# 0xEigenLabs/eigen-zeth

Measured on AMD Instinct MI355X. Metric: goldilocks_ntt_field_elems_per_s, higher is better.
Workload: dtype u64; 1 GPU; forward NTT, natural order in/out, 2^24 rows x 64 columns per GPU (column-major u64), BASELINE configs[3] shape on one GPU; logn=24, cols_per_gpu=64, cols_total=64

## Files before the change

eigen_zeth_amd/csrc/capi.hip:

```cpp
#include <hip/hip_runtime.h>

#include <cstdio>
#include <cstring>
#include <new>
#include <vector>

#include "ctx.hpp"
#include "poseidon_default_table.inc"

extern "C" {

const char *zp_version(void) { return "zethprover-mi355x 0.1 (gfx950)"; }

int32_t zp_device_count(void) {
    int n = 0;
    return hipGetDeviceCount(&n) == hipSuccess ? n : 0;
}

int32_t zp_create(zp_ctx **out, int32_t device) {
    if (!out) return ZP_ERR_ARG;
    *out = nullptr;
    int ndev = 0;
    if (hipGetDeviceCount(&ndev) != hipSuccess || ndev <= 0) return ZP_ERR_HIP;
    if (device < 0 || device >= ndev) return ZP_ERR_ARG;
// ... 341 lines not shown
        u64 a = next(), b = next();
        if (n_bind > 4) a = bind[4];
        if (n_bind > 5) b = bind[5];
        h_pub[4] = a;
        h_pub[5] = b;
        for (size_t i = 0; i < N; i++) {
            fa[i] = a;
            fb[i] = b;
            const u64 t = gl_add(a, b);
            a = b;
            b = t;
        }
        h_pub[6] = fb[N - 1];
        const int k = logn < 16 ? logn : 16;
        const int rep = logn - k;
        h_pub[7] = ((u64)1 << k) - 1;
        for (size_t i = 0; i < N; i++) {
            rv[i] = next() & (((u64)1 << k) - 1);
            tv[i] = (u64)(i >> rep);
            mv[i] = 0;
        }
        for (size_t i = 0; i < N; i++) {
            mv[(size_t)rv[i] << rep] += 1;
            qv[i] = rv[(5 * i + 3) & (N - 1)];
            cv[i] = gl_mul(rv[i], rv[i]);
            dv[i] = gl_add(gl_mul(fa[i], rv[i]), fb[i]);
        }
        return ZP_OK;
    }
    return ZP_ERR_ARG;
}

int32_t zp_ntt_host(zp_ctx *ctx, uint64_t *h_cols, int32_t logn, int32_t W, int32_t inverse) {
    if (!ctx) return ZP_ERR_ARG;
    ZP_BIND(ctx);
    ZP_ARG(ctx, h_cols != nullptr || W == 0, "null host pointer");
    ZP_ARG(ctx, logn >= 0 && logn <= 32 && W >= 0, "logn/W out of range");
    if (W == 0) return ZP_OK;
    const size_t bytes = ((size_t)W << logn) * sizeof(u64);
    void *d = nullptr;
    ZP_TRY(zp_dev_alloc(ctx, bytes, &d));
    int32_t rc = zp_h2d(ctx, d, h_cols, bytes);
    if (rc == ZP_OK) {
        NttRunOpts o;
        rc = zpi_ntt_run(ctx, (u64 *)d, (u64 *)d, logn, W, inverse != 0, o);
    }
    if (rc == ZP_OK) rc = zp_d2h(ctx, h_cols, d, bytes);
    (void)zp_dev_free(ctx, d);
    return rc;
}

int32_t zp_lde_host(zp_ctx *ctx, const uint64_t *h_in, uint64_t *h_out, int32_t logn, int32_t logb,
                    int32_t W, uint64_t shift) {
    if (!ctx) return ZP_ERR_ARG;
    ZP_BIND(ctx);
    ZP_ARG(ctx, (h_in && h_out) || W == 0, "null host pointer");
    ZP_ARG(ctx, logn >= 0 && logb >= 0 && logn + logb <= 32 && W >= 0, "logn/logb/W out of range");
    if (W == 0) return ZP_OK;
    const size_t bin = ((size_t)W << logn) * sizeof(u64), bout = bin << logb;
    void *di = nullptr, *dout = nullptr;
    ZP_TRY(zp_dev_alloc(ctx, bin, &di));
    int32_t rc = zp_dev_alloc(ctx, bout, &dout);
    if (rc == ZP_OK) rc = zp_h2d(ctx, di, h_in, bin);
    if (rc == ZP_OK) rc = zp_lde(ctx, (const uint64_t *)di, (uint64_t *)dout, nullptr, logn, logb, W, shift);
    if (rc == ZP_OK) rc = zp_d2h(ctx, h_out, dout, bout);
    (void)zp_dev_free(ctx, di);
    (void)zp_dev_free(ctx, dout);
    return rc;
}

int32_t zp_set_tuning(zp_ctx *ctx, const char *key, int32_t value) {
    if (!ctx) return ZP_ERR_ARG;
    ZP_ARG(ctx, key != nullptr, "null key");
    if (!strcmp(key, "ntt_logt")) ctx->tune_logt = value;
    else if (!strcmp(key, "ntt_tpw")) ctx->tune_tpw = value;
    else if (!strcmp(key, "ntt_logt9")) ctx->tune_logt9 = value;
    else if (!strcmp(key, "ntt_logt12")) ctx->tune_logt12 = value;
    else if (!strcmp(key, "msm_chunk_log")) ctx->tune_msm_chunk_log = value;
    else if (!strcmp(key, "msm_c")) ctx->tune_msm_c = value;
    else if (!strcmp(key, "ntt_chunk_log")) ctx->tune_ntt_chunk_log = value;
    else if (!strcmp(key, "ntt_maxl")) ctx->tune_ntt_maxl = value;
    else if (!strcmp(key, "ntt_order")) ctx->tune_ntt_order = value;
    else if (!strcmp(key, "ntt_tw1")) ctx->tune_ntt_tw1 = value;
    else if (!strcmp(key, "ntt_limb")) ctx->tune_ntt_limb = value;
    else if (!strcmp(key, "lde_seam")) ctx->tune_lde_seam = value;
    else if (!strcmp(key, "g16_parallel")) ctx->tune_g16_parallel = value;
    else if (!strcmp(key, "seam_tpw")) ctx->tune_seam_tpw = value;
    else if (!strcmp(key, "lde_seam_plans")) ctx->tune_lde_seam_plans = value;
    else if (!strcmp(key, "merkle_top_wave")) ctx->tune_merkle_top_wave = value;
    else if (!strcmp(key, "ntt_small_wave")) ctx->tune_ntt_small_wave = value;
    else if (!strcmp(key, "synth_rowwise")) ctx->tune_synth_rowwise = value;
    else if (!strcmp(key, "p254_scaled")) ctx->tune_p254_scaled = value;
    else if (!strcmp(key, "p254_block")) ctx->tune_p254_block = value;
    else if (!strcmp(key, "fri_fold_lanes")) ctx->tune_fri_fold_lanes = value;
    else if (!strcmp(key, "copy_grid")) ctx->tune_copy_grid = value;
    else if (!strcmp(key, "copy_nt")) ctx->tune_copy_nt = value;
    else if (!strcmp(key, "copy_block")) ctx->tune_copy_block = value;
    else if (!strcmp(key, "copy_unroll")) ctx->tune_copy_unroll = value;
    else if (!strcmp(key, "merkle_coop_log")) ctx->tune_merkle_coop_log = value;
    else if (!strcmp(key, "p254_bulk_log")) ctx->tune_p254_bulk_log = value;
    else if (!strcmp(key, "verify_lane_min")) ctx->tune_verify_lane_min = value;
    else { ctx->err = "unknown tuning key"; return ZP_ERR_ARG; }
    return ZP_OK;
}

int32_t zp_set_profiling(zp_ctx *ctx, int32_t on) {
    if (!ctx) return ZP_ERR_ARG;
    ctx->profiling = on != 0;
    return ZP_OK;
}

int32_t zp_get_pass_timings(zp_ctx *ctx, float *ms, int32_t *radix_log, int32_t cap, int32_t *count) {
    if (!ctx) return ZP_ERR_ARG;
    ZP_BIND(ctx);
    ZP_ARG(ctx, count != nullptr && cap >= 0 && (cap == 0 || (ms && radix_log)), "bad arguments");
    ZP_HIP(ctx, hipStreamSynchronize(ctx->stream));
    int n = 0;
    for (auto &ev : ctx->pass_events) {
        if (n < cap) {
            float t = 0.f;
            ZP_HIP(ctx, hipEventElapsedTime(&t, ev.a, ev.b));
            ms[n] = t;
            radix_log[n] = ev.radix_log;
            n++;
        }
        (void)hipEventDestroy(ev.a);
        (void)hipEventDestroy(ev.b);
    }
    ctx->pass_events.clear();
    *count = n;
    return ZP_OK;
}

int32_t zp_stage_timings(zp_ctx *ctx, char *buf, size_t buflen) {
    if (!ctx) return ZP_ERR_ARG;
    ZP_BIND(ctx);
    ZP_ARG(ctx, buf && buflen > 2, "null buffer");
    ZP_HIP(ctx, hipStreamSynchronize(ctx->stream));
    std::string s = "[";
    bool first = true;
    for (auto &ev : ctx->stage_events) {
        float t = 0.f;
        if (hipEventElapsedTime(&t, ev.a, ev.b) == hipSuccess) {
            char tmp[128];
            snprintf(tmp, sizeof(tmp), "%s{\"stage\": \"%s\", \"ms\": %.4f}", first ? "" : ", ", ev.name, t);
            s += tmp;
            first = false;
        }
        (void)hipEventDestroy(ev.a);
        (void)hipEventDestroy(ev.b);
    }
    ctx->stage_events.clear();
    s += "]";
    ZP_ARG(ctx, s.size() + 1 <= buflen, "buffer too small");
    memcpy(buf, s.c_str(), s.size() + 1);
    return ZP_OK;
}

int32_t zp_ntt_plan_json(zp_ctx *ctx, int32_t logn, char *buf, size_t buflen) {
    if (!ctx) return ZP_ERR_ARG;
    ZP_ARG(ctx, buf && buflen > 0, "null buffer");
    NttPlan *pl;
    ZP_TRY(zpi_get_plan(ctx, logn, false, &pl));
    std::string s = "{\"logn\": " + std::to_string(logn) + ", \"passes\": [";
    for (int i = 0; i < pl->npass; i++) {
        const NttPassShape sh = zpi_plan_pass_shape(ctx, pl, i);
// ... 37 lines not shown
```

eigen_zeth_amd/csrc/ctx.hpp:

```cpp
#pragma once
#include <hip/hip_runtime.h>

#include <map>
#include <string>
#include <vector>

#include "../../include/zeth_prover.h"
#include "gl.hpp"

#define ZP_ROOT32_DEFAULT 1753635133440165772ULL
#define ZP_SHIFT_DEFAULT 49ULL

struct NttPass {
    int L;
    int logPprev;
};

struct NttPlan {
    int logn = 0;
    bool inverse = false;
    int npass = 0;
    NttPass pass[6];
    int lb = 0;
    u64 *d_twl = nullptr;
    u64 *d_twh = nullptr;
    u64 *d_tws = nullptr;
    u64 *d_tw1 = nullptr;
    bool tw1_unavailable = false;
    u64 w16[8];
    u64 ninv = 1;
    int j0inv = 0;
};

struct CosetTable {
    int logn = 0, lb = 0;
    u64 shift = 0, pre = 0;
    u64 *d_lo = nullptr, *d_hi = nullptr;
};

struct ZpG16Cache;
struct zp_ctx {
    int device = 0;
    hipStream_t stream = nullptr;
    hipStream_t own_stream = nullptr;
    std::string err;
    u64 root32 = ZP_ROOT32_DEFAULT;
    u64 coset_shift = ZP_SHIFT_DEFAULT;
    u64 h_rc[360];
    u64 h_mds[144];
    u64 *d_rc = nullptr;
    u32 *d_mds = nullptr;
    bool poseidon_dirty = true;
    bool mds_is_default = false;
    std::map<int, NttPlan> plans;
    std::vector<CosetTable> cosets;
    u64 *scratch[6] = {nullptr, nullptr, nullptr, nullptr, nullptr, nullptr};
    size_t scratch_elems[6] = {0, 0, 0, 0, 0, 0};
    bool ood_valid = false;
    int ood_logn = -1;
    u64 ood_y[3] = {0, 0, 0}, ood_root32 = 0;
    void *pinned = nullptr;
    size_t pinned_bytes = 0;
    zp_ctx *msm_helpers[4] = {nullptr, nullptr, nullptr, nullptr};
    ZpG16Cache *g16_cache = nullptr;
    int num_cu = 256;
    void *msm_arena = nullptr;
    size_t msm_arena_bytes = 0;
    int tune_logt12 = 2;
    int tune_logt = 4, tune_tpw = 2, tune_logt9 = 4;
    int tune_ntt_tw1 = 26;
    int tune_ntt_limb = 0;
    int tune_lde_seam = 1;
    int tune_seam_tpw = 2;
    int tune_copy_grid = 0, tune_copy_nt = 1, tune_copy_block = 0, tune_copy_unroll = 0;
    int tune_lde_seam_plans = 1;
    int tune_g16_parallel = 1;
    int tune_ntt_order = 0;
    int tune_ntt_maxl = 0;
    int tune_ntt_small_wave = 0;
    int tune_fri_fold_lanes = 0;
    int tune_synth_rowwise = 0;
    int tune_p254_block = 0;
    int tune_p254_scaled = 0;
    int tune_merkle_top_wave = 0;
    int tune_merkle_coop_log = 0;
    int tune_ntt_chunk_log = 0;
    int tune_p254_bulk_log = 0;
    int tune_msm_c = 0;
    int tune_verify_lane_min = 0;
    int tune_msm_chunk_log = 0;
    std::multimap<size_t, void *> prove_pool;
    size_t prove_pool_bytes = 0;
    std::map<std::string, u64 *> prove_fixed;
    size_t prove_fixed_bytes = 0;
    std::map<std::string, void *> air_kernels;
    struct DigestEntry { std::vector<uint64_t> words; uint8_t dg[32]; };
    std::vector<DigestEntry> digest_cache;
    std::vector<u64> last_openings;
    bool profiling = false;
    struct PassEv { hipEvent_t a, b; int radix_log; };
    std::vector<PassEv> pass_events;
    struct StageEv { hipEvent_t a, b; const char *name; };
    std::vector<StageEv> stage_events;
};

struct ZpStage {
    zp_ctx *ctx;
    zp_ctx::StageEv ev;
    bool on;
    ZpStage(zp_ctx *c, const char *name) : ctx(c), on(c && c->profiling) {
        if (c) (void)hipSetDevice(c->device);
        if (on) {
            ev.name = name;
            on = hipEventCreate(&ev.a) == hipSuccess && hipEventCreate(&ev.b) == hipSuccess &&
                 hipEventRecord(ev.a, ctx->stream) == hipSuccess;
        }
    }
    ~ZpStage() {
        if (on && hipEventRecord(ev.b, ctx->stream) == hipSuccess) ctx->stage_events.push_back(ev);
    }
};

#define ZP_BIND(ctx) do { if (ctx) (void)hipSetDevice((ctx)->device); } while (0)

#define ZP_HIP(ctx, call)                                                                    \
    do {                                                                                     \
        hipError_t e_ = (call);                                                              \
        if (e_ != hipSuccess) {                                                              \
            (ctx)->err = std::string(#call) + ": " + hipGetErrorString(e_);                  \
            return e_ == hipErrorOutOfMemory ? ZP_ERR_NOMEM : ZP_ERR_HIP;                    \
        }                                                                                    \
    } while (0)

#define ZP_ARG(ctx, cond, msg)                                                               \
    do {                                                                                     \
        if (!(cond)) {                                                                       \
            (ctx)->err = std::string("bad argument: ") + (msg);                              \
            return ZP_ERR_ARG;                                                               \
        }                                                                                    \
    } while (0)

#define ZP_TRY(expr)                                                                         \
    do {                                                                                     \
        int32_t rc_ = (expr);                                                                \
        if (rc_ != ZP_OK) return rc_;                                                        \
    } while (0)

int32_t zpi_scratch(zp_ctx *ctx, int which, size_t elems, u64 **out);
int32_t zpi_pinned(zp_ctx *ctx, size_t bytes, void **out);
int32_t zpi_d2h_small(zp_ctx *ctx, void *h_dst, const void *d_src, size_t bytes);
int32_t zpi_h2d_small(zp_ctx *ctx, void *d_dst, const void *h_src, size_t bytes);
int32_t zpi_upload(zp_ctx *ctx, const std::vector<u64> &h, u64 **d);
// ... 44 lines not shown
```

eigen_zeth_amd/csrc/ntt.hip:

```cpp
#include <hip/hip_runtime.h>

#include <cstring>
#include <string>

#include "ctx.hpp"
#include "wave_xchg.hpp"
#include "gl_asm.hpp"
#include "gl_limb.hpp"

#define ZP_LDG(p) __builtin_nontemporal_load(p)
#define ZP_STG(p, v) __builtin_nontemporal_store(v, p)

namespace {

typedef __attribute__((ext_vector_type(4))) int zp_i32x4;

struct PassArgs {
    const u64 *in;
    u64 *out;
    u64 in_cs, out_cs;
    u64 in_valid;
    const u64 *twl, *twh;
    const u64 *tws;
    const u64 *tw1;
    const u64 *csl, *csh;
    u64 scale;
    int logn, logPprev, lb, cslb;
    int j0inv;
    int flags;
    int ncols;
};

__device__ __forceinline__ constexpr int brev(int x, int bits) {
    int r = 0;
    for (int i = 0; i < bits; i++) r |= ((x >> i) & 1) << (bits - 1 - i);
    return r;
}
__device__ __forceinline__ constexpr int slot_of(int o, int j, int pos, int A) {
    return ((o >> pos) << (pos + A)) | (j << pos) | (o & ((1 << pos) - 1));
}

template <int A1, int A2, int A3, int LOGT>
struct Geo {
    static constexpr int L = A1 + A2 + A3;
    static constexpr int R = 1 << L;
    static constexpr int T = 1 << LOGT;
    static constexpr int LT = LOGT;
    static constexpr int NT = (R * T) / 16;
    static constexpr int J = 1 + (A2 > 0 ? 1 : 0) + (A3 > 0 ? 1 : 0);
    static constexpr int POS1 = L - A1;
    static constexpr int POS2 = L - A1 - A2;
    static constexpr int AJ = (J == 1) ? A1 : (J == 2 ? A2 : A3);
    __device__ static __forceinline__ int kof(int sigma) {
        int k = (sigma >> POS1) & ((1 << A1) - 1);
        if (A2 > 0) k |= ((sigma >> POS2) & ((1 << A2) - 1)) << A1;
        if (A3 > 0) k |= (sigma & ((1 << A3) - 1)) << (A1 + A2);
        return k;
    }
    __device__ static __forceinline__ int sigma_of_k(int k) {
        int s = (k & ((1 << A1) - 1)) << POS1;
        if (A2 > 0) s |= ((k >> A1) & ((1 << A2) - 1)) << POS2;
        if (A3 > 0) s |= (k >> (A1 + A2)) & ((1 << A3) - 1);
        return s;
    }
    __device__ static __forceinline__ int lpos(int sigma, int t) {
        int s2 = sigma;
        if constexpr (LOGT < 4 && A3 > 0) {
            constexpr int GB = 5 - LOGT;
            s2 ^= ((sigma >> POS2) & ((1 << GB) - 1)) ^ (((sigma >> (POS1 + LOGT)) & ((1 << (A1 - LOGT)) - 1)) << 1);
        }
        return (s2 << LOGT) + (t ^ (kof(sigma) & (T - 1)));
    }
};

__device__ __forceinline__ u64 tw_lookup(const u64 *lo, const u64 *hi, int lb, u64 e) {
    u64 a = lo[e & ((1ULL << lb) - 1)];
    u64 b = hi[e >> lb];
    return gl_mul(a, b);
}

__device__ __forceinline__ u64 mul_c16(int e, u64 d) {
    switch (e) {
        case 0: return d;
        case 1: return gl_shl12<1>(d);
        case 2: return gl_shl12<2>(d);
        case 3: return gl_shl12<3>(d);
        case 4: return gl_shl12<4>(d);
        case 5: return gl_shl12<5>(d);
        case 6: return gl_shl12<6>(d);
        default: return gl_shl12<7>(d);
    }
}
template <int A>
__device__ __forceinline__ void dif_shift(u64 *v) {
    static_assert(A >= 2 && A <= 4, "radix 4, 8 or 16");
#pragma unroll
    for (int s = 0; s < A; s++) {
        const int half = 1 << (A - 1 - s);
#pragma unroll
        for (int t = 0; t < (1 << (A - 1)); t += 2) {
            const int i0 = (t / half) * 2 * half + (t % half), i1 = ((t + 1) / half) * 2 * half + ((t + 1) % half);
            gl_bfly2(v[i0], v[i0 + half], v[i1], v[i1 + half]);
            v[i0 + half] = mul_c16((t % half) * (8 / half), v[i0 + half]);
            v[i1 + half] = mul_c16(((t + 1) % half) * (8 / half), v[i1 + half]);
        }
    }
}

__device__ __forceinline__ void lds_barrier() {
    __builtin_amdgcn_fence(__ATOMIC_RELEASE, "workgroup", "local");
    __builtin_amdgcn_s_barrier();
    __builtin_amdgcn_fence(__ATOMIC_ACQUIRE, "workgroup", "local");
}
// ... 46 lines not shown
        case 1: return gl_l4_mul_c16<1>(d);
        case 2: return gl_l4_mul_c16<2>(d);
        case 3: return gl_l4_mul_c16<3>(d);
        case 4: return gl_l4_mul_c16<4>(d);
        case 5: return gl_l4_mul_c16<5>(d);
        case 6: return gl_l4_mul_c16<6>(d);
        default: return gl_l4_mul_c16<7>(d);
    }
}
template <int A>
__device__ __forceinline__ void dif_levels_l4(gl_l4 *x) {
    static_assert(A >= 2 && A <= 4, "radix 4, 8 or 16");
#pragma unroll
    for (int s = 0; s < A; s++) {
        const int half = 1 << (A - 1 - s);
#pragma unroll
        for (int t = 0; t < (1 << (A - 1)); t++) {
            const int i0 = (t / half) * 2 * half + (t % half);
            const gl_l4 a = x[i0], b = x[i0 + half];
            x[i0] = gl_l4_add(a, b);
            x[i0 + half] = mul_c16_l4((t % half) * (8 / half), gl_l4_sub(a, b));
        }
    }
}
template <int A>
__device__ __forceinline__ void dif_shift_l4(const u64 *v, gl_l4 *x) {
#pragma unroll
    for (int i = 0; i < (1 << A); i++) x[i] = gl_l4_from(v[i]);
    dif_levels_l4<A>(x);
}
__device__ __forceinline__ gl_w4 w4_load(const gl_w4 *p) {
    const zp_i32x4 a = *(const zp_i32x4 *)p->lo, b = *(const zp_i32x4 *)p->hi;
    gl_w4 w;
    w.lo[0] = a.x; w.lo[1] = a.y; w.lo[2] = a.z; w.lo[3] = a.w;
    w.hi[0] = b.x; w.hi[1] = b.y; w.hi[2] = b.z; w.hi[3] = b.w;
    return w;
}
__device__ __forceinline__ void w4_store(gl_w4 *p, const u64 w0, const u64 w1, const u64 w2, const u64 w3) {
    i32 l[4], h[4];
    gl_l4_balance(w0, l[0], h[0]);
    gl_l4_balance(w1, l[1], h[1]);
    gl_l4_balance(w2, l[2], h[2]);
    gl_l4_balance(w3, l[3], h[3]);
    zp_i32x4 a = {l[0], l[1], l[2], l[3]}, b = {h[0], h[1], h[2], h[3]};
    *(zp_i32x4 *)p->lo = a;
    *(zp_i32x4 *)p->hi = b;
}
template <typename G, int A, int POS, int ANEXT, int POSNEXT>
__device__ __forceinline__ void exchange2_l4(const gl_l4 *x, u64 *v, u64 *lds, const gl_w4 *twr4, int j0inv, int tid) {
    constexpr int GR = 16 >> A;
#pragma unroll
    for (int g = 0; g < GR; g++) {
        const int gamma = g * G::NT + tid;
        const int t = gamma & (G::T - 1), o = gamma >> G::LT;
        const int rho = o & ((1 << POS) - 1);
#pragma unroll
        for (int p = 0; p < (1 << A); p++) {
            const int kj = (j0inv * brev(p, A)) & ((1 << A) - 1);
            const u64 y = p == 0 ? gl_l4_canon(x[g * (1 << A)]) : gl_l4_mul(x[g * (1 << A) + p], w4_load(twr4 + kj * rho));
            lds[G::lpos(slot_of(o, kj, POS, A), t)] = y;
        }
    }
    lds_barrier();
    exchange_read<G, ANEXT, POSNEXT>(v, lds, tid);
}

template <typename G>
__device__ __forceinline__ void table_copy_out(u64 *v, const u64 *lds, const u64 *twb, u64 *blk, int tid) {
    constexpr int L = G::L, NT = G::NT;
#pragma unroll
    for (int i = 0; i < 16; i++) v[i] = twb[i * NT + tid];
    lds_barrier();
#pragma unroll
    for (int i = 0; i < 16; i += 2) {
        const int ia = i * NT + tid, ib = (i + 1) * NT + tid;
        u64 xa = lds[G::lpos(G::sigma_of_k(ia & ((1 << L) - 1)), ia >> L)];
        u64 xb = lds[G::lpos(G::sigma_of_k(ib & ((1 << L) - 1)), ib >> L)];
        gl_mul2(xa, v[i], xb, v[i + 1]);
        ZP_STG(&blk[ia], xa);
        ZP_STG(&blk[ib], xb);
    }
}

template <int A1, int A2, int A3, int LOGT, bool TRANSPOSE, bool PADDED, int MODE, bool BIG = false, bool LIMB = false>
__global__ void __launch_bounds__((1 << (A1 + A2 + A3 + LOGT)) / 16, LIMB ? 3 : 4)
ntt_pass2_kernel(PassArgs a, int tiles_per_wg) {
    using G = Geo<A1, A2, A3, LOGT>;
    constexpr int L = G::L, R = G::R, T = G::T, NT = G::NT, AJ = G::AJ;
    constexpr int GRJ = 16 >> AJ;
    constexpr int R2 = 1 << (A2 + A3);
    constexpr bool HAS_TAB = !TRANSPOSE && MODE >= 1;
    constexpr bool TWR_LDS = L <= 10;
    constexpr int TPL = (R + NT - 1) / NT;
    extern __shared__ __attribute__((aligned(16))) u64 lds[];
    constexpr int REC = LIMB ? 4 : 1;
    u64 *tab = lds + R * T;
    u64 *twr1 = tab + (HAS_TAB ? R * REC : 0);
    u64 *twr2 = twr1 + R * REC;
    constexpr bool TW1 = TRANSPOSE && MODE == 3;
    static_assert(!LIMB || (TWR_LDS && (TW1 || !TRANSPOSE)), "limb form: LDS twiddle copies, no per-lane twiddle chain");
    u64 col = blockIdx.y, wg_lin = blockIdx.x;
    if constexpr (TW1) {
        const u64 x = blockIdx.x & 7u, j = blockIdx.x >> 3;
        col = j % (u64)a.ncols;
        wg_lin = (j / (u64)a.ncols) * 8 + x;
    }
    const int logNR = a.logn - L;
    const int logP = a.logPprev;
    const u64 N = 1ULL << a.logn;
    const u64 *src = a.in + col * a.in_cs;
    u64 *dst = a.out + col * a.out_cs;
    u64 v[16], vn[16];
    constexpr int NTW = TW1 ? 1 : TRANSPOSE ? (GRJ + 2) : (MODE == 2 ? TPL + 1 : TPL);
    u64 twl_c[NTW], twh_c[NTW], twl_n[NTW], twh_n[NTW];

    constexpr bool small_n = !BIG;
    auto fetch_tile = [&](u64 *r, u64 *tl, u64 *th, u64 u0, int tid) {
        constexpr int GR = 16 >> A1;
        const u64 valid_rows = a.in_valid >> logNR;
#pragma unroll
        for (int g = 0; g < GR; g++) {
            const int gamma = g * NT + tid;
            const int t = gamma & (T - 1), o = gamma >> LOGT;
            const u32 slot0 = (u32)slot_of(o, 0, G::POS1, A1);
            const u32 lane_bytes = (((u32)slot0 << logNR) + (u32)t) << 3;
            const u64 lane_el = ((u64)slot0 << logNR) + (u64)t;
#pragma unroll
            for (int j = 0; j < (1 << A1); j++) {
                const u64 *rowp = src + (((u64)j << G::POS1) << logNR) + u0;
                const u64 *ptr;
                if constexpr (small_n) ptr = (const u64 *)((const char *)rowp + lane_bytes);
                else ptr = rowp + lane_el;
                u64 val;
                if constexpr (PADDED) val = (u64)(slot0 + ((u32)j << G::POS1)) < valid_rows ? (LOGT < 4 ? *ptr : ZP_LDG(ptr)) : 0ULL;
                else val = LOGT < 4 ? *ptr : ZP_LDG(ptr);
                r[g * (1 << A1) + j] = val;
            }
        }
        const u64 lm = (1ULL << a.lb) - 1;
        if constexpr (TW1) {
            (void)tl; (void)th; (void)lm;
        } else if constexpr (TRANSPOSE) {
            const int t = tid & (T - 1);
            const u64 u = u0 + t;
            const int jr = a.j0inv & ((1 << AJ) - 1);
            u64 e[NTW];
#pragma unroll
            for (int g = 0; g < GRJ; g++) e[g] = u * (u64)G::kof(((g * NT + tid) >> LOGT) << AJ);
            e[GRJ] = ((u << (L - AJ)) * (u64)jr) & (N - 1);
            e[GRJ + 1] = (N - ((u << L) & (N - 1))) & (N - 1);
#pragma unroll
            for (int i = 0; i < NTW; i++) { tl[i] = a.twl[e[i] & lm]; th[i] = a.twh[e[i] >> a.lb]; }
        } else {
            if constexpr (MODE >= 1) {
                const u64 e0 = (u0 >> logP) << logP;
#pragma unroll
                for (int j = 0; j < TPL; j++) {
                    const u64 e = (a.flags & 1) ? e0 * (u64)((tid + j * NT) & (R - 1)) : 0;
                    tl[j] = a.twl[e & lm];
                    th[j] = a.twh[e >> a.lb];
                }
            }
            if constexpr (MODE == 2) {
                const u64 c = (u0 + (tid & (T - 1))) & ((1ULL << logP) - 1);
                tl[TPL] = a.csl[c & ((1ULL << a.cslb) - 1)];
                th[TPL] = a.csh[c >> a.cslb];
            }
        }
    };

    u64 wg = wg_lin;
    if constexpr (LOGT < 4 && !TW1) {
        if ((gridDim.x & 7u) == 0) wg = (u64)(blockIdx.x & 7u) * (gridDim.x >> 3) + (blockIdx.x >> 3);
    }
    const u64 tile0 = wg * tiles_per_wg;
    fetch_tile(v, twl_c, twh_c, tile0 << LOGT, threadIdx.x);
    u64 kfac[TPL];
    {
        const int tid0 = threadIdx.x;
        if constexpr (LIMB) {
            for (int e = tid0; e < R; e += NT) {
                const int rot = (a.j0inv * (R / 8)) & (R - 1);
                w4_store((gl_w4 *)twr1 + e, a.tws[e << (12 - L)], a.tws[((e + rot) & (R - 1)) << (12 - L)],
                         a.tws[((e + 2 * rot) & (R - 1)) << (12 - L)], a.tws[((e + 3 * rot) & (R - 1)) << (12 - L)]);
            }
            if constexpr (G::J >= 3) {
                constexpr int L2 = A2 + A3;
                for (int e = tid0; e < R2; e += NT) {
                    const int rot = (a.j0inv * (R2 / 8)) & (R2 - 1);
                    w4_store((gl_w4 *)twr2 + e, a.tws[e << (12 - L2)], a.tws[((e + rot) & (R2 - 1)) << (12 - L2)],
                             a.tws[((e + 2 * rot) & (R2 - 1)) << (12 - L2)], a.tws[((e + 3 * rot) & (R2 - 1)) << (12 - L2)]);
                }
            }
        } else if constexpr (TWR_LDS) {
            if (tid0 < R) twr1[tid0] = a.tws[tid0 << (12 - L)];
            if constexpr (G::J >= 3) {
                if (tid0 < R2) twr2[tid0] = a.tws[tid0 << (12 - (A2 + A3))];
            }
        }
#pragma unroll
        for (int j = 0; j < TPL; j++) {
            kfac[j] = 1;
            if constexpr (HAS_TAB) {
                if (a.flags & 2) kfac[j] = a.scale;
                if constexpr (MODE == 2) {
                    const u64 ek = (u64)((tid0 + j * NT) & (R - 1)) << logP;
                    kfac[j] = gl_mul(kfac[j], gl_mul(a.csl[ek & ((1ULL << a.cslb) - 1)], a.csh[ek >> a.cslb]));
                }
            }
        }
    }
    lds_barrier();
    __builtin_amdgcn_s_waitcnt(0x0F70);
#pragma clang loop unroll(disable)
    for (int it = 0; it < tiles_per_wg; it++) {
        const u64 u0 = (tile0 + it) << LOGT;
        const bool more = it + 1 < tiles_per_wg;
        int tid = threadIdx.x;
        asm volatile("" : "+v"(tid));
        if (more) fetch_tile(vn, twl_n, twh_n, u0 + T, tid);

        const u64 s = TRANSPOSE ? 0 : (u0 >> logP);
        if constexpr (HAS_TAB) {
#pragma unroll
            for (int j = 0; j < TPL; j++)
                if (tid + j * NT < R) {
                    const u64 w = gl_mul(gl_mul(twl_c[j], twh_c[j]), kfac[j]);
                    if constexpr (LIMB) w4_store((gl_w4 *)tab + tid + j * NT, w, gl_shl12<2>(w), gl_shl12<4>(w), gl_shl12<6>(w));
                    else tab[tid + j * NT] = w;
                }
        }
        gl_l4 x[LIMB ? 16 : 1];
        if constexpr (LIMB) {
#pragma unroll
            for (int g = 0; g < (16 >> A1); g++) dif_shift_l4<A1>(v + g * (1 << A1), x + g * (1 << A1));
            exchange2_l4<G, A1, G::POS1, A2, G::POS2>(x, v, lds, (const gl_w4 *)twr1, a.j0inv, tid);
#pragma unroll
            for (int g = 0; g < (16 >> A2); g++) dif_shift_l4<A2>(v + g * (1 << A2), x + g * (1 << A2));
            if constexpr (G::J >= 3) {
                exchange2_l4<G, A2, G::POS2, A3, 0>(x, v, lds, (const gl_w4 *)twr2, a.j0inv, tid);
#pragma unroll
                for (int g = 0; g < (16 >> A3); g++) dif_shift_l4<A3>(v + g * (1 << A3), x + g * (1 << A3));
            }
        } else {
#pragma unroll
        for (int g = 0; g < (16 >> A1); g++) dif_shift<A1>(v + g * (1 << A1));
        exchange2<G, A1, G::POS1, A2, G::POS2, TWR_LDS ? 0 : 12 - L>(v, lds, TWR_LDS ? twr1 : a.tws, a.j0inv, tid);
#pragma unroll
        for (int g = 0; g < (16 >> A2); g++) dif_shift<A2>(v + g * (1 << A2));
        if constexpr (G::J >= 3) {
            exchange2<G, A2, G::POS2, A3, 0, TWR_LDS ? 0 : 12 - (A2 + A3)>(v, lds, TWR_LDS ? twr2 : a.tws, a.j0inv, tid);
#pragma unroll
            for (int g = 0; g < (16 >> A3); g++) dif_shift<A3>(v + g * (1 << A3));
        }
        }
#pragma unroll
        for (int g = 0; g < GRJ; g++) {
            const int gamma = g * NT + tid;
            const int t = gamma & (T - 1), o = gamma >> LOGT;
            const int klow = G::kof(o << AJ);
            if constexpr (TW1) {
                const int jr = a.j0inv & ((1 << AJ) - 1);
#pragma unroll
                for (int i = 0; i < (1 << AJ); i++) {
                    const int kj = (jr * i) & ((1 << AJ) - 1);
                    if constexpr (LIMB) lds[G::lpos(slot_of(o, kj, 0, AJ), t)] = gl_l4_canon(x[g * (1 << AJ) + brev(i, AJ)]);
                    else lds[G::lpos(slot_of(o, kj, 0, AJ), t)] = v[g * (1 << AJ) + brev(i, AJ)];
                }
            } else if constexpr (TRANSPOSE) {
                const int jr = a.j0inv & ((1 << AJ) - 1);
                u64 w = gl_mul(twl_c[g], twh_c[g]);
                const u64 hj = gl_mul(twl_c[GRJ], twh_c[GRJ]);
                const u64 hjd = gl_mul(hj, gl_mul(twl_c[GRJ + 1], twh_c[GRJ + 1]));
#pragma unroll
                for (int i = 0; i < (1 << AJ); i++) {
                    const int p = brev(i, AJ);
                    const int kj = (jr * i) & ((1 << AJ) - 1);
                    u64 x = v[g * (1 << AJ) + p];
                    if (i + 1 < (1 << AJ)) {
                        const bool wrap = ((jr * (i + 1)) >> AJ) != ((jr * i) >> AJ);
                        u64 wn = w;
                        gl_mul2(x, w, wn, wrap ? hjd : hj);
                        w = wn;
                    } else {
                        x = gl_mul1(x, w);
                    }
                    lds[G::lpos(slot_of(o, kj, 0, AJ), t)] = x;
                }
            } else {
                u64 *const sbase = dst + (s << (logP + L)) + (u0 & ((1ULL << logP) - 1));
                const u32 lane_sb = (((u32)klow << logP) + (u32)t) << 3;
                const u64 lane_se = ((u64)klow << logP) + (u64)t;
                u64 cw = 1;
                if constexpr (MODE == 2) cw = gl_mul(twl_c[TPL], twh_c[TPL]);
#pragma unroll
                for (int p = 0; p < (1 << AJ); p += 2) {
                    const int kja = (a.j0inv * brev(p, AJ)) & ((1 << AJ) - 1), kjb = (a.j0inv * brev(p + 1, AJ)) & ((1 << AJ) - 1);
                    const int ka = klow + (kja << (L - AJ)), kb = klow + (kjb << (L - AJ));
                    u64 xa, xb;
                    if constexpr (LIMB) {
                        if constexpr (MODE >= 1) {
                            xa = gl_l4_mul(x[g * (1 << AJ) + p], w4_load((const gl_w4 *)tab + ka));
                            xb = gl_l4_mul(x[g * (1 << AJ) + p + 1], w4_load((const gl_w4 *)tab + kb));
                        } else {
                            xa = gl_l4_canon(x[g * (1 << AJ) + p]);
                            xb = gl_l4_canon(x[g * (1 << AJ) + p + 1]);
                        }
                    } else {
                        xa = v[g * (1 << AJ) + p];
                        xb = v[g * (1 << AJ) + p + 1];
                        if constexpr (MODE >= 1) gl_mul2(xa, tab[ka], xb, tab[kb]);
                    }
                    if constexpr (MODE == 2) gl_mul2(xa, cw, xb, cw);
                    u64 *const ua = sbase + ((u64)(kja << (L - AJ)) << logP), *const ub = sbase + ((u64)(kjb << (L - AJ)) << logP);
                    u64 *pa, *pb;
                    if constexpr (small_n) { pa = (u64 *)((char *)ua + lane_sb); pb = (u64 *)((char *)ub + lane_sb); }
                    else { pa = ua + lane_se; pb = ub + lane_se; }
                    if constexpr (LOGT < 4) {
                        *pa = xa;
                        *pb = xb;
                    } else {
                        ZP_STG(pa, xa);
                        ZP_STG(pb, xb);
                    }
                }
            }
        }
        if constexpr (TW1) {
            table_copy_out<G>(v, lds, a.tw1 + (u0 << L), dst + (u0 << L), tid);
        } else if constexpr (TRANSPOSE) {
            lds_barrier();
            u64 *blk = dst + (u0 << L);
#pragma unroll
            for (int i = 0; i < 16; i++) {
                const int idx = i * NT + tid;
                const int t2 = idx >> L, k = idx & ((1 << L) - 1);
                ZP_STG(&blk[idx], lds[G::lpos(G::sigma_of_k(k), t2)]);
            }
        }
        if (more) {
            lds_barrier();
#pragma unroll
            for (int i = 0; i < 16; i++) v[i] = vn[i];
#pragma unroll
            for (int i = 0; i < NTW; i++) { twl_c[i] = twl_n[i]; twh_c[i] = twh_n[i]; }
        }
    }
}

struct SeamArgs {
    const u64 *in;
    u64 *out;
    u64 *coef;
    const u64 *tws_i, *tws_f;
    const u64 *tw1;
    const u64 *csl, *csh;
    u64 scale;
    int logn, cslb, j0inv_i, j0inv_f, ncols;
};
__global__ void __launch_bounds__(256, 4) lde_seam_kernel(SeamArgs a, int tiles_per_wg) {
    using G = Geo<4, 4, 0, 4>;
    constexpr int L = 8, R = 256, T = 16, LOGT = 4;
    extern __shared__ __attribute__((aligned(16))) u64 lds[];
    u64 *tab = lds + R * T;
    u64 *twr_i = tab + R;
    u64 *twr_f = twr_i + R;
    const u64 x8 = blockIdx.x & 7u, jj = blockIdx.x >> 3;
    const u64 col = jj % (u64)a.ncols, wg = (jj / (u64)a.ncols) * 8 + x8;
    const int logNR = a.logn - L;
    const u64 N = 1ULL << a.logn;
    const u64 *src = a.in + col * N;
    u64 *dst = a.out + col * (2 * N);
    u64 *cdst = a.coef ? a.coef + col * N : nullptr;
    u64 v[16];
    u64 cw_c[2];
    auto fetch_tile = [&](u64 *r, u64 *cwr, u64 u0, int tid) {
        const int t = tid & (T - 1), o = tid >> LOGT;
        const u32 slot0 = (u32)slot_of(o, 0, G::POS1, 4);
        const u32 lane_bytes = (((u32)slot0 << logNR) + (u32)t) << 3;
#pragma unroll
        for (int j = 0; j < 16; j++) {
            const u64 *rowp = src + (((u64)j << G::POS1) << logNR) + u0;
            r[j] = ZP_LDG((const u64 *)((const char *)rowp + lane_bytes));
        }
        const u64 c = u0 + (u64)t;
        cwr[0] = a.csl[c & ((1ULL << a.cslb) - 1)];
        cwr[1] = a.csh[c >> a.cslb];
    };
    const u64 tile0 = wg * tiles_per_wg;
    {
        const int tid0 = threadIdx.x;
        twr_i[tid0] = a.tws_i[tid0 << (12 - L)];
        twr_f[tid0] = a.tws_f[tid0 << (12 - L)];
        const u64 ek = (u64)tid0 << logNR;
        tab[tid0] = gl_mul(a.scale, gl_mul(a.csl[ek & ((1ULL << a.cslb) - 1)], a.csh[ek >> a.cslb]));
    }
    lds_barrier();
#pragma clang loop unroll(disable)
    for (int it = 0; it < tiles_per_wg; it++) {
        const u64 u0 = (tile0 + it) << LOGT;
        int tid = threadIdx.x;
        asm volatile("" : "+v"(tid));
        fetch_tile(v, cw_c, u0, tid);
        const int t = tid & (T - 1), o = tid >> LOGT;
        dif_shift<4>(v);
        exchange2<G, 4, G::POS1, 4, G::POS2, 0>(v, lds, twr_i, a.j0inv_i, tid);
        dif_shift<4>(v);
        const u64 cw = gl_mul(cw_c[0], cw_c[1]);
        lds_barrier();
#pragma unroll
        for (int p = 0; p < 16; p += 2) {
            const int kja = (a.j0inv_i * brev(p, 4)) & 15, kjb = (a.j0inv_i * brev(p + 1, 4)) & 15;
            const int ka = o + (kja << 4), kb = o + (kjb << 4);
            u64 xa = v[p], xb = v[p + 1];
            gl_mul2(xa, tab[ka], xb, tab[kb]);
            gl_mul2(xa, cw, xb, cw);
            if (cdst) {
                ZP_STG((u64 *)((char *)(cdst + ((u64)ka << logNR) + u0) + (t << 3)), xa);
                ZP_STG((u64 *)((char *)(cdst + ((u64)kb << logNR) + u0) + (t << 3)), xb);
            }
            lds[(((ka & 1) << 7) + (ka >> 1)) * T + t] = xa;
            lds[(((kb & 1) << 7) + (kb >> 1)) * T + t] = xb;
        }
        lds_barrier();
        u64 f1[8];
#pragma unroll
        for (int j = 0; j < 8; j++) {
            v[j] = lds[((j << 4) + o) * T + t];
            f1[j] = lds[(128 + (j << 4) + o) * T + t];
        }
// ... 43 lines not shown
    if (!((lane >> LH) & 1)) return gl_add(x, y);
    const u64 d = gl_sub(y, x);
    return i ? gl_mul(d, tws[(u64)i << (12 - (LH + 1))]) : d;
}

template <bool WAVE>
__global__ void __launch_bounds__(256) ntt_small_kernel(SmallArgs a) {
    extern __shared__ __attribute__((aligned(16))) u64 lds[];
    const int tid = threadIdx.x;
    const int n = 1 << a.logn;
    const u64 *src = a.in + (u64)blockIdx.x * a.in_cs;
    u64 *dst = a.out + (u64)blockIdx.x * a.out_cs;
    for (int i = tid; i < n; i += 256) lds[i] = (u64)i < a.in_valid ? src[i] : 0ULL;
    __syncthreads();
    const int lds_stages = WAVE ? (a.logn > 6 ? a.logn - 6 : 0) : a.logn;
    for (int s = 0; s < lds_stages; s++) {
        const int lh = a.logn - 1 - s;
        const int half = 1 << lh;
        for (int b = tid; b < (n >> 1); b += 256) {
            const int i = b & (half - 1);
            const int i0 = ((b >> lh) << (lh + 1)) + i, i1 = i0 + half;
            u64 x = lds[i0], y = lds[i1];
            lds[i0] = gl_add(x, y);
            u64 d = gl_sub(x, y);
            lds[i1] = i ? gl_mul(d, a.tws[(u64)i << (12 - (lh + 1))]) : d;
        }
        __syncthreads();
    }
    if constexpr (WAVE) {
        const int lane = tid & 63;
        for (int base = (tid >> 6) << 6; base < n; base += 256) {
            u64 x = base + lane < n ? lds[base + lane] : 0ULL;
            const int top = a.logn < 6 ? a.logn : 6;
            if (top >= 6) x = wave_stage<5>(x, lane, a.tws);
            if (top >= 5) x = wave_stage<4>(x, lane, a.tws);
            if (top >= 4) x = wave_stage<3>(x, lane, a.tws);
            if (top >= 3) x = wave_stage<2>(x, lane, a.tws);
            if (top >= 2) x = wave_stage<1>(x, lane, a.tws);
            if (top >= 1) x = wave_stage<0>(x, lane, a.tws);
            const int i = base + lane;
            if (i < n) {
                const int k = brev(i, a.logn);
                if (a.flags & 2) x = gl_mul(x, a.scale);
                if (a.flags & 4) x = gl_mul(x, tw_lookup(a.csl, a.csh, a.cslb, (u64)k));
                dst[k] = x;
            }
        }
        return;
    }
    for (int i = tid; i < n; i += 256) {
        const int k = brev(i, a.logn);
        u64 x = lds[i];
        if (a.flags & 2) x = gl_mul(x, a.scale);
        if (a.flags & 4) x = gl_mul(x, tw_lookup(a.csl, a.csh, a.cslb, (u64)k));
        dst[k] = x;
    }
}

__global__ void __launch_bounds__(256) coset_scale_kernel(const u64 *in, u64 *out, u64 n, const u64 *lo,
                                                         const u64 *hi, int lb) {
    const u64 col = blockIdx.y;
    const u64 i = ((u64)blockIdx.x * 256 + threadIdx.x);
    if (i < n) out[col * n + i] = gl_mul(in[col * n + i], tw_lookup(lo, hi, lb, i));
}

__global__ void __launch_bounds__(256) twiddle_rows_kernel(u64 *rows, int logn_row, u64 total, u64 row0, u64 nmask,
                                                           const u64 *lo, const u64 *hi, int lb) {
    const u64 i = (u64)blockIdx.x * 256 + threadIdx.x;
    if (i >= total) return;
    const u64 r = i >> logn_row, k = i & ((1ULL << logn_row) - 1);
    const u64 e = ((row0 + r) * k) & nmask;
    rows[i] = gl_mul(rows[i], tw_lookup(lo, hi, lb, e));
}

__global__ void __launch_bounds__(256) tw1_fill_kernel(u64 *out, int logn, int L, const u64 *lo, const u64 *hi, int lb) {
    const u64 i = (u64)blockIdx.x * 256 + threadIdx.x;
    if (i >> logn) return;
    const u64 u = i >> L, k = i & ((1ULL << L) - 1);
    out[i] = tw_lookup(lo, hi, lb, (u * k) & ((1ULL << logn) - 1));
}

using PassKernel = void (*)(PassArgs, int);

template <int A1, int A2, int A3, int LOGT, bool BIG>
PassKernel pick_pass_kernel(bool transpose, bool table, bool padded, int mode, bool limb) {
    constexpr bool CAN_TABLE = !BIG && A3 == 0, CAN_LIMB = !BIG && A1 + A2 + A3 <= 8;
    if constexpr (CAN_TABLE) {
        if (table && limb) return padded ? ntt_pass2_kernel<A1, A2, A3, LOGT, true, true, 3, false, CAN_LIMB> : ntt_pass2_kernel<A1, A2, A3, LOGT, true, false, 3, false, CAN_LIMB>;
        if (table) return padded ? ntt_pass2_kernel<A1, A2, A3, LOGT, true, true, 3, false> : ntt_pass2_kernel<A1, A2, A3, LOGT, true, false, 3, false>;
    }
    if (transpose) return padded ? ntt_pass2_kernel<A1, A2, A3, LOGT, true, true, 1, BIG> : ntt_pass2_kernel<A1, A2, A3, LOGT, true, false, 1, BIG>;
    if (limb) return mode == 2 ? ntt_pass2_kernel<A1, A2, A3, LOGT, false, false, 2, BIG, CAN_LIMB>
                   : mode == 1 ? ntt_pass2_kernel<A1, A2, A3, LOGT, false, false, 1, BIG, CAN_LIMB>
                               : ntt_pass2_kernel<A1, A2, A3, LOGT, false, false, 0, BIG, CAN_LIMB>;
    return mode == 2 ? ntt_pass2_kernel<A1, A2, A3, LOGT, false, false, 2, BIG>
         : mode == 1 ? ntt_pass2_kernel<A1, A2, A3, LOGT, false, false, 1, BIG>
                     : ntt_pass2_kernel<A1, A2, A3, LOGT, false, false, 0, BIG>;
}

template <int A1, int A2, int A3, int LOGT, bool BIG = false>
int32_t launch_pass2(zp_ctx *ctx, PassArgs a, bool transpose, int W) {
    using G = Geo<A1, A2, A3, LOGT>;
    const u64 tiles = (1ULL << (a.logn - G::L)) >> LOGT;
    int tpw = ctx->tune_tpw;
    while (tpw > 1 && (tiles % tpw != 0 || tiles / tpw * (u64)W < (u64)ctx->num_cu * 4)) tpw >>= 1;
    dim3 grid((unsigned)(tiles / tpw), (unsigned)W), block(G::NT);
    const bool table = !BIG && A3 == 0 && transpose && a.tw1 && (grid.x & 7u) == 0;
    const int mode = transpose ? 0 : (a.flags & 4) ? 2 : (a.flags & 3) ? 1 : 0;
    const bool limb = !BIG && G::L <= 8 && ctx->tune_ntt_limb != 0 && (!transpose || table);
    const size_t rec = limb ? 4 : 1;
    const size_t shmem = ((size_t)G::R * G::T + (mode >= 1 ? G::R * rec : 0) + (G::L <= 10 ? (G::R + (1 << (A2 + A3))) * rec : 0)) * sizeof(u64);
    const PassKernel k = pick_pass_kernel<A1, A2, A3, LOGT, BIG>(transpose, table, a.in_valid != (1ULL << a.logn), mode, limb);
    if (shmem > 65536) ZP_HIP(ctx, hipFuncSetAttribute((const void *)k, hipFuncAttributeMaxDynamicSharedMemorySize, (int)shmem));
    if (table) {
        a.ncols = W;
        grid = dim3(grid.x * (unsigned)W);
    }
    hipLaunchKernelGGL(k, grid, block, shmem, ctx->stream, a, tpw);
    ZP_HIP(ctx, hipGetLastError());
    return ZP_OK;
}

constexpr int shape_key(int A1, int A2, int A3, int logT, bool big) { return (((A1 * 8 + A2) * 8 + A3) * 8 + logT) * 2 + big; }

int32_t dispatch_pass(zp_ctx *ctx, const NttPass &p, const PassArgs &a, bool transpose, int W) {
    const bool big = a.logn > 28;
    const NttPassShape s = zpi_pass_shape(ctx, p.L, big, transpose, (a.flags & 7) != 0);
#define ZP_PASS_SHAPE(A1, A2, A3, LOGT, BIG) case shape_key(A1, A2, A3, LOGT, BIG): return launch_pass2<A1, A2, A3, LOGT, BIG>(ctx, a, transpose, W)
    switch (shape_key(s.A1, s.A2, s.A3, s.logT, big)) {
        ZP_PASS_SHAPE(3, 2, 0, 5, false);
        ZP_PASS_SHAPE(3, 3, 0, 5, false);
        ZP_PASS_SHAPE(4, 3, 0, 5, false);
        ZP_PASS_SHAPE(4, 3, 0, 5, true);
        ZP_PASS_SHAPE(4, 4, 0, 4, false);
        ZP_PASS_SHAPE(4, 4, 0, 4, true);
        ZP_PASS_SHAPE(4, 4, 0, 5, false);
        ZP_PASS_SHAPE(3, 3, 3, 4, false);
        ZP_PASS_SHAPE(3, 3, 3, 5, false);
        ZP_PASS_SHAPE(4, 3, 3, 4, false);
        ZP_PASS_SHAPE(4, 4, 3, 3, false);
        ZP_PASS_SHAPE(4, 4, 4, 1, false);
        ZP_PASS_SHAPE(4, 4, 4, 2, false);
        default: ctx->err = big ? "pass radix not built for transforms above 2^28 rows" : "unsupported pass radix"; return ZP_ERR_UNSUPPORTED;
    }
#undef ZP_PASS_SHAPE
}

struct PassTimer {
    zp_ctx *ctx;
    zp_ctx::PassEv ev;
    bool on;
    PassTimer(zp_ctx *c, int radix_log) : ctx(c), on(c->profiling) {
        ev.radix_log = radix_log;
        on = on && hipEventCreate(&ev.a) == hipSuccess && hipEventCreate(&ev.b) == hipSuccess && hipEventRecord(ev.a, ctx->stream) == hipSuccess;
    }
    ~PassTimer() {
        if (on && hipEventRecord(ev.b, ctx->stream) == hipSuccess) ctx->pass_events.push_back(ev);
    }
};

template <typename Args>
void set_output_scaling(Args &a, bool inverse, const CosetTable *post_scale) {
    if (inverse) a.flags |= 2;
    if (post_scale) {
        a.flags |= 4;
        a.csl = post_scale->d_lo;
        a.csh = post_scale->d_hi;
        a.cslb = post_scale->lb;
    }
}

int chunk_columns(const zp_ctx *ctx, int logn, int W) {
    const int wc = (int)((1ULL << (ctx->tune_ntt_chunk_log > 0 ? ctx->tune_ntt_chunk_log : 28)) >> logn);
    return wc < 1 ? 1 : wc > W ? W : wc;
}

}

NttPassShape zpi_pass_shape(const zp_ctx *ctx, int L, bool big, bool transpose, bool multiplies) {
    static const NttPassShape by_l[8] = {{3, 2, 0, 5}, {3, 3, 0, 5}, {4, 3, 0, 5}, {4, 4, 0, 4}, {3, 3, 3, 4}, {4, 3, 3, 4}, {4, 4, 3, 3}, {4, 4, 4, 2}};
    if (L < 5 || L > 12 || (big && L != 7 && L != 8)) return {0, 0, 0, 0};
    NttPassShape s = by_l[L - 5];
    if (big) return s;
    if ((L == 8 && ctx->tune_logt != 4) || (L == 9 && ctx->tune_logt9 != 4)) s.logT = 5;
    if (L == 12 && ctx->tune_logt12 == 1 && (transpose || !multiplies)) s.logT = 1;
    return s;
}

NttPassShape zpi_plan_pass_shape(const zp_ctx *ctx, const NttPlan *pl, int i) {
    return zpi_pass_shape(ctx, pl->pass[i].L, pl->logn > 28, i == 0, i + 1 < pl->npass || pl->inverse);
}

static int32_t upload_power_table(zp_ctx *ctx, int logn, u64 base, u64 pre, int *lb, u64 **d_lo, u64 **d_hi) {
    *lb = (logn + 1) / 2;
    std::vector<u64> lo(1ULL << *lb), hi(1ULL << (logn - *lb));
    lo[0] = pre;
    u64 sp = 1;
    for (size_t i = 1; i < lo.size(); i++) {
        sp = gl_mul(sp, base);
        lo[i] = gl_mul(pre, sp);
// ... 338 lines not shown
```

Before: 95.45 billion field-elems/s.

## Add TileWalk tile mapping and optional persistent NTT pass kernels

Moves the mapping of workgroups to (column, tile group) into a TileWalk helper that supports several orders and a 1D grid. It adds an optional persistent kernel variant that strides over work items and prefetches the next column's tile across group boundaries. It also skips the kfac multiply when the mode does not need it. Persistence is off by default and the default order matches the old mapping, so the default path mainly changes indexing overhead and the kfac multiply.

```diff
diff --git a/eigen_zeth_amd/csrc/capi.hip b/eigen_zeth_amd/csrc/capi.hip
--- a/eigen_zeth_amd/csrc/capi.hip
+++ b/eigen_zeth_amd/csrc/capi.hip
@@ -447,6 +447,8 @@
     else if (!strcmp(key, "ntt_maxl")) ctx->tune_ntt_maxl = value;
     else if (!strcmp(key, "ntt_order")) ctx->tune_ntt_order = value;
     else if (!strcmp(key, "ntt_tw1")) ctx->tune_ntt_tw1 = value;
+    else if (!strcmp(key, "ntt_tile_map")) ctx->tune_ntt_tile_map = value;
+    else if (!strcmp(key, "ntt_persist")) ctx->tune_ntt_persist = value;
     else if (!strcmp(key, "ntt_limb")) ctx->tune_ntt_limb = value;
     else if (!strcmp(key, "lde_seam")) ctx->tune_lde_seam = value;
     else if (!strcmp(key, "g16_parallel")) ctx->tune_g16_parallel = value;
diff --git a/eigen_zeth_amd/csrc/ctx.hpp b/eigen_zeth_amd/csrc/ctx.hpp
--- a/eigen_zeth_amd/csrc/ctx.hpp
+++ b/eigen_zeth_amd/csrc/ctx.hpp
@@ -68,6 +68,8 @@
     size_t msm_arena_bytes = 0;
     int tune_logt12 = 2;
     int tune_logt = 4, tune_tpw = 2, tune_logt9 = 4;
+    int tune_ntt_tile_map = 0;
+    int tune_ntt_persist = 0;
     int tune_ntt_tw1 = 26;
     int tune_ntt_limb = 0;
     int tune_lde_seam = 1;
diff --git a/eigen_zeth_amd/csrc/ntt.hip b/eigen_zeth_amd/csrc/ntt.hip
--- a/eigen_zeth_amd/csrc/ntt.hip
+++ b/eigen_zeth_amd/csrc/ntt.hip
@@ -29,6 +29,41 @@
     int j0inv;
     int flags;
     int ncols;
+    int walk;
+    unsigned step_hi, step_lo;
+};
+constexpr int WALK_GRID1D = 4;
+
+struct TileWalk {
+    unsigned hi, lo;
+    static __device__ __forceinline__ int order(const PassArgs &a) { return a.walk & 3; }
+    static __device__ __forceinline__ int log_groups(const PassArgs &a) { return a.walk >> 8; }
+    __device__ __forceinline__ void start(const PassArgs &a) {
+        lo = blockIdx.x;
+        hi = blockIdx.y;
+        if (order(a) == 2) {
+            const unsigned j = blockIdx.x >> 3;
+            hi = j / (unsigned)a.ncols;
+            lo = j - hi * (unsigned)a.ncols;
+        } else if (a.walk & WALK_GRID1D) {
+            hi = blockIdx.x >> log_groups(a);
+            lo = blockIdx.x & ((1u << log_groups(a)) - 1);
+        }
+    }
+    __device__ __forceinline__ bool step(const PassArgs &a) {
+        const unsigned m = order(a) == 2 ? (unsigned)a.ncols : 1u << log_groups(a);
+        lo += a.step_lo;
+        hi += a.step_hi;
+        if (lo >= m) {
+            lo -= m;
+            hi++;
+        }
+        return hi < (order(a) == 2 ? 1u << (log_groups(a) - 3) : (unsigned)a.ncols);
+    }
+    __device__ __forceinline__ unsigned group(const PassArgs &a) const {
+        return order(a) == 2 ? hi * 8 + (blockIdx.x & 7u) : order(a) == 1 ? ((lo & 7u) << (log_groups(a) - 3)) + (lo >> 3) : lo;
+    }
+    __device__ __forceinline__ unsigned col(const PassArgs &a) const { return order(a) == 2 ? lo : hi; }
 };
 
 __device__ __forceinline__ constexpr int brev(int x, int bits) {
@@ -241,9 +276,8 @@
     }
 }
 
-template <int A1, int A2, int A3, int LOGT, bool TRANSPOSE, bool PADDED, int MODE, bool BIG = false, bool LIMB = false>
-__global__ void __launch_bounds__((1 << (A1 + A2 + A3 + LOGT)) / 16, LIMB ? 3 : 4)
-ntt_pass2_kernel(PassArgs a, int tiles_per_wg) {
+template <int A1, int A2, int A3, int LOGT, bool TRANSPOSE, bool PADDED, int MODE, bool BIG, bool LIMB, bool PERSIST>
+__device__ __forceinline__ void pass2_body(const PassArgs &a, int tiles_per_wg) {
     using G = Geo<A1, A2, A3, LOGT>;
     constexpr int L = G::L, R = G::R, T = G::T, NT = G::NT, AJ = G::AJ;
     constexpr int GRJ = 16 >> AJ;
@@ -258,24 +292,20 @@
     u64 *twr2 = twr1 + R * REC;
     constexpr bool TW1 = TRANSPOSE && MODE == 3;
     static_assert(!LIMB || (TWR_LDS && (TW1 || !TRANSPOSE)), "limb form: LDS twiddle copies, no per-lane twiddle chain");
-    u64 col = blockIdx.y, wg_lin = blockIdx.x;
-    if constexpr (TW1) {
-        const u64 x = blockIdx.x & 7u, j = blockIdx.x >> 3;
-        col = j % (u64)a.ncols;
-        wg_lin = (j / (u64)a.ncols) * 8 + x;
-    }
+    TileWalk walk;
+    walk.start(a);
+    unsigned col = walk.col(a);
     const int logNR = a.logn - L;
     const int logP = a.logPprev;
     const u64 N = 1ULL << a.logn;
-    const u64 *src = a.in + col * a.in_cs;
-    u64 *dst = a.out + col * a.out_cs;
     u64 v[16], vn[16];
     constexpr int NTW = TW1 ? 1 : TRANSPOSE ? (GRJ + 2) : (MODE == 2 ? TPL + 1 : TPL);
     u64 twl_c[NTW], twh_c[NTW], twl_n[NTW], twh_n[NTW];
 
     constexpr bool small_n = !BIG;
-    auto fetch_tile = [&](u64 *r, u64 *tl, u64 *th, u64 u0, int tid) {
+    auto fetch_tile = [&](u64 *r, u64 *tl, u64 *th, u64 fcol, u64 u0, int tid) {
         constexpr int GR = 16 >> A1;
+        const u64 *src = a.in + fcol * a.in_cs;
         const u64 valid_rows = a.in_valid >> logNR;
 #pragma unroll
         for (int g = 0; g < GR; g++) {
@@ -328,12 +358,8 @@
         }
     };
 
-    u64 wg = wg_lin;
-    if constexpr (LOGT < 4 && !TW1) {
-        if ((gridDim.x & 7u) == 0) wg = (u64)(blockIdx.x & 7u) * (gridDim.x >> 3) + (blockIdx.x >> 3);
-    }
-    const u64 tile0 = wg * tiles_per_wg;
-    fetch_tile(v, twl_c, twh_c, tile0 << LOGT, threadIdx.x);
+    unsigned tile0 = walk.group(a) * tiles_per_wg;
+    fetch_tile(v, twl_c, twh_c, col, (u64)tile0 << LOGT, threadIdx.x);
     u64 kfac[TPL];
     {
         const int tid0 = threadIdx.x;
@@ -373,18 +399,28 @@
     __builtin_amdgcn_s_waitcnt(0x0F70);
 #pragma clang loop unroll(disable)
     for (int it = 0; it < tiles_per_wg; it++) {
-        const u64 u0 = (tile0 + it) << LOGT;
-        const bool more = it + 1 < tiles_per_wg;
+        const u64 u0 = (u64)(tile0 + it) << LOGT;
+        u64 *const dst = a.out + col * a.out_cs;
+        bool more = it + 1 < tiles_per_wg;
+        unsigned ntile = tile0 + it + 1, ncol = col;
+        if constexpr (PERSIST) {
+            if (!more && walk.step(a)) {
+                more = true;
+                ntile = walk.group(a) * tiles_per_wg;
+                ncol = walk.col(a);
+            }
+        }
         int tid = threadIdx.x;
         asm volatile("" : "+v"(tid));
-        if (more) fetch_tile(vn, twl_n, twh_n, u0 + T, tid);
+        if (more) fetch_tile(vn, twl_n, twh_n, ncol, (u64)ntile << LOGT, tid);
 
         const u64 s = TRANSPOSE ? 0 : (u0 >> logP);
         if constexpr (HAS_TAB) {
 #pragma unroll
             for (int j = 0; j < TPL; j++)
                 if (tid + j * NT < R) {
-                    const u64 w = gl_mul(gl_mul(twl_c[j], twh_c[j]), kfac[j]);
+                    u64 w = gl_mul(twl_c[j], twh_c[j]);
+                    if (MODE == 2 || (a.flags & 2)) w = gl_mul(w, kfac[j]);
                     if constexpr (LIMB) w4_store((gl_w4 *)tab + tid + j * NT, w, gl_shl12<2>(w), gl_shl12<4>(w), gl_shl12<6>(w));
                     else tab[tid + j * NT] = w;
                 }
@@ -504,7 +540,25 @@
 #pragma unroll
             for (int i = 0; i < NTW; i++) { twl_c[i] = twl_n[i]; twh_c[i] = twh_n[i]; }
         }
-    }
+        if constexpr (PERSIST) {
+            if (more && it + 1 == tiles_per_wg) {
+                tile0 = walk.group(a) * tiles_per_wg;
+                col = walk.col(a);
+                it = -1;
+            }
+        }
+    }
+}
+
+template <int A1, int A2, int A3, int LOGT, bool TRANSPOSE, bool PADDED, int MODE, bool BIG = false, bool LIMB = false>
+__global__ void __launch_bounds__((1 << (A1 + A2 + A3 + LOGT)) / 16, LIMB ? 3 : 4)
+ntt_pass2_kernel(PassArgs a, int tiles_per_wg) {
+    pass2_body<A1, A2, A3, LOGT, TRANSPOSE, PADDED, MODE, BIG, LIMB, false>(a, tiles_per_wg);
+}
+template <int A1, int A2, int A3, int LOGT, bool TRANSPOSE, bool PADDED, int MODE, bool BIG = false, bool LIMB = false>
+__global__ void __launch_bounds__((1 << (A1 + A2 + A3 + LOGT)) / 16, LIMB ? 3 : 4)
+ntt_pass2_persist_kernel(PassArgs a, int tiles_per_wg) {
+    pass2_body<A1, A2, A3, LOGT, TRANSPOSE, PADDED, MODE, BIG, LIMB, true>(a, tiles_per_wg);
 }
 
 struct SeamArgs {
@@ -714,20 +768,26 @@
 
 using PassKernel = void (*)(PassArgs, int);
 
-template <int A1, int A2, int A3, int LOGT, bool BIG>
+template <bool P, int A1, int A2, int A3, int LOGT, bool TRANSPOSE, bool PADDED, int MODE, bool BIG, bool LIMB>
+constexpr PassKernel pass_k() {
+    if constexpr (P) return ntt_pass2_persist_kernel<A1, A2, A3, LOGT, TRANSPOSE, PADDED, MODE, BIG, LIMB>;
+    else return ntt_pass2_kernel<A1, A2, A3, LOGT, TRANSPOSE, PADDED, MODE, BIG, LIMB>;
+}
+
+template <int A1, int A2, int A3, int LOGT, bool BIG, bool P = false>
 PassKernel pick_pass_kernel(bool transpose, bool table, bool padded, int mode, bool limb) {
     constexpr bool CAN_TABLE = !BIG && A3 == 0, CAN_LIMB = !BIG && A1 + A2 + A3 <= 8;
     if constexpr (CAN_TABLE) {
-        if (table && limb) return padded ? ntt_pass2_kernel<A1, A2, A3, LOGT, true, true, 3, false, CAN_LIMB> : ntt_pass2_kernel<A1, A2, A3, LOGT, true, false, 3, false, CAN_LIMB>;
-        if (table) return padded ? ntt_pass2_kernel<A1, A2, A3, LOGT, true, true, 3, false> : ntt_pass2_kernel<A1, A2, A3, LOGT, true, false, 3, false>;
-    }
-    if (transpose) return padded ? ntt_pass2_kernel<A1, A2, A3, LOGT, true, true, 1, BIG> : ntt_pass2_kernel<A1, A2, A3, LOGT, true, false, 1, BIG>;
-    if (limb) return mode == 2 ? ntt_pass2_kernel<A1, A2, A3, LOGT, false, false, 2, BIG, CAN_LIMB>
-                   : mode == 1 ? ntt_pass2_kernel<A1, A2, A3, LOGT, false, false, 1, BIG, CAN_LIMB>
-                               : ntt_pass2_kernel<A1, A2, A3, LOGT, false, false, 0, BIG, CAN_LIMB>;
-    return mode == 2 ? ntt_pass2_kernel<A1, A2, A3, LOGT, false, false, 2, BIG>
-         : mode == 1 ? ntt_pass2_kernel<A1, A2, A3, LOGT, false, false, 1, BIG>
-                     : ntt_pass2_kernel<A1, A2, A3, LOGT, false, false, 0, BIG>;
+        if (table && limb) return padded ? pass_k<P, A1, A2, A3, LOGT, true, true, 3, false, CAN_LIMB>() : pass_k<P, A1, A2, A3, LOGT, true, false, 3, false, CAN_LIMB>();
+        if (table) return padded ? pass_k<P, A1, A2, A3, LOGT, true, true, 3, false, false>() : pass_k<P, A1, A2, A3, LOGT, true, false, 3, false, false>();
+    }
+    if (transpose) return padded ? pass_k<P, A1, A2, A3, LOGT, true, true, 1, BIG, false>() : pass_k<P, A1, A2, A3, LOGT, true, false, 1, BIG, false>();
+    if (limb) return mode == 2 ? pass_k<P, A1, A2, A3, LOGT, false, false, 2, BIG, CAN_LIMB>()
+                   : mode == 1 ? pass_k<P, A1, A2, A3, LOGT, false, false, 1, BIG, CAN_LIMB>()
+                               : pass_k<P, A1, A2, A3, LOGT, false, false, 0, BIG, CAN_LIMB>();
+    return mode == 2 ? pass_k<P, A1, A2, A3, LOGT, false, false, 2, BIG, false>()
+         : mode == 1 ? pass_k<P, A1, A2, A3, LOGT, false, false, 1, BIG, false>()
+                     : pass_k<P, A1, A2, A3, LOGT, false, false, 0, BIG, false>();
 }
 
 template <int A1, int A2, int A3, int LOGT, bool BIG = false>
@@ -736,18 +796,34 @@
     const u64 tiles = (1ULL << (a.logn - G::L)) >> LOGT;
     int tpw = ctx->tune_tpw;
     while (tpw > 1 && (tiles % tpw != 0 || tiles / tpw * (u64)W < (u64)ctx->num_cu * 4)) tpw >>= 1;
-    dim3 grid((unsigned)(tiles / tpw), (unsigned)W), block(G::NT);
+    const u64 groups = tiles / tpw;
+    dim3 grid((unsigned)groups, (unsigned)W), block(G::NT);
     const bool table = !BIG && A3 == 0 && transpose && a.tw1 && (grid.x & 7u) == 0;
     const int mode = transpose ? 0 : (a.flags & 4) ? 2 : (a.flags & 3) ? 1 : 0;
     const bool limb = !BIG && G::L <= 8 && ctx->tune_ntt_limb != 0 && (!transpose || table);
     const size_t rec = limb ? 4 : 1;
     const size_t shmem = ((size_t)G::R * G::T + (mode >= 1 ? G::R * rec : 0) + (G::L <= 10 ? (G::R + (1 << (A2 + A3))) * rec : 0)) * sizeof(u64);
-    const PassKernel k = pick_pass_kernel<A1, A2, A3, LOGT, BIG>(transpose, table, a.in_valid != (1ULL << a.logn), mode, limb);
+    a.ncols = W;
+    int log_groups = 0;
+    while ((1ULL << log_groups) < groups) log_groups++;
+    const bool by8 = (groups & 7u) == 0;
+    const int tm = ctx->tune_ntt_tile_map;
+    const int order = !by8 ? 0 : tm == 3 ? 1 : table ? 2 : (tm == 1 || tm == 2) ? tm : LOGT < 4 ? 1 : 0;
+    const u64 items = groups * (u64)W;
+    u64 cap = ctx->tune_ntt_persist > 0 && !BIG ? (u64)ctx->tune_ntt_persist * (u64)ctx->num_cu : 0;
+    if (order == 2) cap &= ~7ULL;
+    const bool persist = cap != 0 && cap < items, grid1d = order == 2 || persist;
+    a.walk = order | (grid1d ? WALK_GRID1D : 0) | (log_groups << 8);
+    if (grid1d) grid = dim3((unsigned)(persist ? cap : items));
+    const u64 stride = (persist ? cap : 0) >> (order == 2 ? 3 : 0), m = order == 2 ? (u64)W : groups;
+    a.step_hi = (unsigned)(stride / m);
+    a.step_lo = (unsigned)(stride % m);
+    const bool padded = a.in_valid != (1ULL << a.logn);
+    PassKernel k = pick_pass_kernel<A1, A2, A3, LOGT, BIG>(transpose, table, padded, mode, limb);
+    if constexpr (!BIG) {
+        if (persist) k = pick_pass_kernel<A1, A2, A3, LOGT, BIG, true>(transpose, table, padded, mode, limb);
+    }
     if (shmem > 65536) ZP_HIP(ctx, hipFuncSetAttribute((const void *)k, hipFuncAttributeMaxDynamicSharedMemorySize, (int)shmem));
-    if (table) {
-        a.ncols = W;
-        grid = dim3(grid.x * (unsigned)W);
-    }
     hipLaunchKernelGGL(k, grid, block, shmem, ctx->stream, a, tpw);
     ZP_HIP(ctx, hipGetLastError());
     return ZP_OK;
```

After: 95.30 billion field-elems/s, median of 2. About the same (-0.2%).
